# facebookresearch/AVID-CMA

Measured on AMD Instinct MI355X. Metric: clips/sec (video+audio fwd+bwd+NCE+Adam), higher is better.
Workload: dtype f32 (bf16x3 MFMA)

## Files before the change

### avid-cma_amd/avid_hip/lib.py

```python
from __future__ import annotations

import ctypes as C
import os
import subprocess


import torch

_HERE = os.path.dirname(os.path.abspath(__file__))
_PKG = os.path.dirname(_HERE)
LIB_PATH = os.environ.get("AVID_HIP_LIB") or os.path.join(_HERE, "libavid_hip.so")

AVID_OK = 0


class BnBwdFuse(C.Structure):
    _fields_ = [("x", C.c_void_p), ("scale", C.c_void_p), ("shift", C.c_void_p), ("mean", C.c_void_p),
                ("invstd", C.c_void_p), ("relu", C.c_int32), ("partials", C.c_void_p)]


class InAffine(C.Structure):
    _fields_ = [("scale", C.c_void_p), ("shift", C.c_void_p), ("relu", C.c_int32)]


# ... 52 lines not shown
_lib = _load()

_vp, _i, _i64, _u64, _f, _sz = C.c_void_p, C.c_int, C.c_int64, C.c_uint64, C.c_float, C.c_size_t
_dp = C.POINTER(ConvDesc)

SIGNATURES = {
    "avid_last_error": (C.c_char_p, []),
    "avid_version": (_i, []),
    "avid_device_info": (_i, [_i, C.POINTER(_i), C.POINTER(_i), C.c_char_p, _i]),
    "avid_timing_enable": (_i, [_i]),
    "avid_timing_report": (_i, [C.c_char_p, _sz]),
    "avid_conv_fwd_workspace_bytes": (_sz, [_dp]),
    "avid_conv_fwd_stats_rows": (_i, [_dp]),
    "avid_conv_fwd": (_i, [_dp, _vp, _vp, _vp, _vp, _vp, _i, _vp, _vp, _vp, _sz, _vp]),
    "avid_conv_takes_in_affine": (_i, [_dp]),
    "avid_conv_fwd_in": (_i, [_dp, _vp, _vp, _vp, _vp, _vp, _vp, _i, _vp, _vp, _vp, _sz, _vp]),
    "avid_debug_in_affine_launches": (C.c_longlong, [_i]),
    "avid_conv_dgrad_workspace_bytes": (_sz, [_dp]),
    "avid_conv_dgrad_bn_rows": (_i, [_dp]),
    "avid_conv_dgrad": (_i, [_dp, _vp, _vp, _vp, _vp, _vp, _vp, _vp, _vp, _vp, _sz, _vp]),
    "avid_weight_transpose_batched": (_i, [_i, _vp, _i64, _vp]),
    "avid_weight_transform": (_i, [_vp, _vp]),
    "avid_conv_wgrad_workspace_bytes": (_sz, [_dp]),
    "avid_conv_wgrad": (_i, [_dp, _vp, _vp, _vp, _vp, _sz, _vp]),
    "avid_conv_wgrad_in": (_i, [_dp, _vp, _vp, _vp, _vp, _vp, _sz, _vp]),
    "avid_conv_wgrad_groupable": (_i, [_dp]),
    "avid_conv_wgrad_group_workspace_bytes": (_sz, [_i, C.POINTER(WgradItem)]),
    "avid_conv_wgrad_group": (_i, [_i, C.POINTER(WgradItem), _vp, _sz, _vp]),
    "avid_conv_kernel_name": (_i, [_dp, _i, C.c_char_p, _i]),
    "avid_conv_uses_wino": (_i, [_dp, _i]),
    "avid_conv_uses_split": (_i, [_dp, _i]),
    "avid_conv_split_bytes": (_sz, [_dp]),
    "avid_debug_presplit_launches": (C.c_longlong, []),
    "avid_wino_configure": (_i, [_i, _i64, _i]),
    "avid_wino2_configure": (_i, [_i]),
    "avid_wino2_pre_configure": (_i, [_i]),
    "avid_wgrad_pre_configure": (_i, [_i]),
    "avid_stem_fwd_pre_configure": (_i, [_i]),
    "avid_tconv_configure": (_i, [_i]),
    "avid_set_cu_budget": (_i, [_i]),
    "avid_cu_budget": (_i, []),
    "avid_bn_workspace_bytes": (_sz, [_i64, _i]),
    "avid_bn_fwd_train": (_i, [_i64, _i, _vp, _vp, _vp, _vp, _vp, _f, _f, _i, _vp, _vp, _vp, _vp, _vp, _vp, _vp, _i, _vp, _sz, _vp]),
    "avid_bn_fwd_eval": (_i, [_i64, _i, _vp, _vp, _vp, _vp, _vp, _f, _i, _vp, _vp, _vp]),
    "avid_bn_bwd": (_i, [_i64, _i, _vp, _vp, _vp, _vp, _vp, _vp, _vp, _i, _vp, _vp, _vp, _vp, _i, _i, _vp, _sz, _vp]),
    "avid_bn_relu_maxpool_fwd": (_i, [_i, _i, _i, _i, _i, _vp, _vp, _vp, _vp, _vp, _f, _f, _vp, _vp, _vp, _vp, _vp, _vp, _vp,
                                      _vp, _i, _vp, _sz, _vp]),
    "avid_bn_relu_maxpool_bwd": (_i, [_i, _i, _i, _i, _i, _vp, _vp, _vp, _vp, _vp, _vp, _vp, _vp, _vp, _vp, _vp, _vp, _sz,
                                      _vp]),
    "avid_clip_normalize": (_i, [_i, _i, _i, _i, _vp, C.POINTER(_f), C.POINTER(_f), _vp, _vp]),
    "avid_logspec_basis_floats": (_sz, [_i]),
    "avid_logspec_basis": (_i, [_i, _vp, _vp]),
    "avid_logspec_workspace_bytes": (_sz, [_i, _i, _i]),
    "avid_logspec": (_i, [_i, _i, _vp, _i, _i, _i, _vp, _vp, _vp, _f, _vp, _vp, _sz, _vp]),
    "avid_maxpool_hw3s2_fwd": (_i, [_i, _i, _i, _i, _i, _vp, _vp, _vp, _vp]),
    "avid_maxpool_hw3s2_bwd": (_i, [_i, _i, _i, _i, _i, _vp, _vp, _vp, _vp]),
    "avid_global_maxpool_fwd": (_i, [_i, _i, _i, _vp, _vp, _vp, _vp]),
    "avid_global_maxpool_bwd": (_i, [_i, _i, _i, _vp, _vp, _vp, _vp]),
    "avid_relu_bwd": (_i, [_i64, _vp, _vp, _vp, _vp]),
    "avid_colsum": (_i, [_i64, _i, _vp, _vp, _vp]),
    "avid_l2norm_fwd": (_i, [_i, _i, _vp, _vp, _vp, _vp]),
    "avid_l2norm_bwd": (_i, [_i, _i, _vp, _vp, _vp, _vp, _vp]),
    "avid_alias_draw": (_i, [_i64, _i64, _vp, _vp, _i, _u64, _u64, _vp, _vp, _i64, _vp, _vp]),
    "avid_counter_add": (_i, [_vp, _u64, _vp]),
    "avid_bank_scores_fwd": (_i, [_i, _i, _i, _i64, _vp, _vp, _vp, _f, _vp, _vp, _vp, _vp]),
    "avid_bank_scores_bwd": (_i, [_i, _i, _i, _i64, _vp, _vp, _vp, _vp, _f, _i, _vp, _vp]),
# ... 86 lines not shown
```

### avid-cma_amd/csrc/conv.hip

```cpp
#include <math.h>
#include <stdlib.h>

#include <atomic>
#include <type_traits>

#include "common.h"

namespace avid {

typedef unsigned int uintx4 __attribute__((ext_vector_type(4)));

struct ConvArgs {
  const float* __restrict__ src;
  const float* __restrict__ wk;
  int w_row, w_nrec;
  const float* __restrict__ addend;
  const float* __restrict__ bias;
  float* __restrict__ dst;
  float* __restrict__ part;
  int B, Ts, Hs, Ws, Cs;
  int Td, Hd, Wd, Cd;
  int kt, kh, kw;
  int st, sh, sw;
  int pt, ph, pw;
// ... 279 lines not shown

constexpr int EPI_ANY = 15;
#ifdef AVID_PK_TRACE
__device__ long long g_pk_trace[1024 * 64];
extern "C" int avid_debug_pk_trace(long long* host) {
  return (int)hipMemcpyFromSymbol(host, HIP_SYMBOL(g_pk_trace), sizeof(long long) * 1024 * 64);
}
#define PK_STAMP(idx) do { if (threadIdx.x == 0 && (idx) < 32) { g_pk_trace[blockIdx.x * 64 + (idx)] = wall_clock64(); g_pk_trace[blockIdx.x * 64 + 32 + (idx)] = clock64(); } } while (0)
#else
#define PK_STAMP(idx) do {} while (0)
#endif
#ifdef AVID_PK_FP32
constexpr bool PK_SPLIT = false;
#else
constexpr bool PK_SPLIT = true;
#endif
typedef __bf16 pk_bf16x8 __attribute__((ext_vector_type(8)));
typedef unsigned pk_uintx4 __attribute__((ext_vector_type(4)));
template <bool DOT = true>
__device__ __forceinline__ void pk_split8(const floatx4& v0, const floatx4& v1, pk_bf16x8& fh, pk_bf16x8& fm, pk_bf16x8& fl) {
  const float v[8] = {v0[0], v0[1], v0[2], v0[3], v1[0], v1[1], v1[2], v1[3]};
  unsigned h[4], m[4], l[4];
#pragma unroll
  for (int i = 0; i < 4; ++i) {
    if (DOT) split2_bf16_dot(v[2 * i], v[2 * i + 1], h[i], m[i], l[i]);
    else split2_bf16(v[2 * i], v[2 * i + 1], h[i], m[i], l[i]);
  }
  fh = __builtin_bit_cast(pk_bf16x8, pk_uintx4{h[0], h[1], h[2], h[3]});
  fm = __builtin_bit_cast(pk_bf16x8, pk_uintx4{m[0], m[1], m[2], m[3]});
  fl = __builtin_bit_cast(pk_bf16x8, pk_uintx4{l[0], l[1], l[2], l[3]});
}

constexpr int PK_BCH = 2 * 2 * 3 * 1024;
template <int WM, int WN, int TM, int TN, int MODE, bool STRIDED = false, int EPI = EPI_ANY, bool BS = false>
__global__ __launch_bounds__(WM * WN * 64, 2) void igemm_pk_kernel(const ConvArgs p) {
  static_assert(!STRIDED || MODE == 1, "parity classes are a dgrad construct");
  constexpr int NT = WM * WN * 64;
  constexpr int BM = WM * TM * 32, BN = WN * TN * 32;
  constexpr int RPP = NT / 8;
  constexpr int PA = BM / RPP, PB = BN / RPP;
  static_assert(BM % RPP == 0 && BN % RPP == 0, "tile rows must be a multiple of the staging pass");
  static_assert(!BS || (NT == 256 && (BN == 64 || BN == 128) && PK_SPLIT), "pre-split weights: the 4-wave tiles of the split-bf16 build");
  constexpr int BCH = (BN / 64) * PK_BCH;
  constexpr int PB3 = BCH / (NT * 16);
  constexpr bool ASWZ = BS && BN == 128;
  constexpr int ALD = ASWZ ? BK : LDK;
  constexpr int STAGE = BS ? BM * ALD + BCH / 4 : (BM + BN) * LDK;
  extern __shared__ __attribute__((aligned(16))) float smem[];
  typedef const ConvArgs __attribute__((address_space(4)))* KArgs;
  const KArgs kp = (KArgs)__builtin_amdgcn_kernarg_segment_ptr();
  const int tid = threadIdx.x, lane = tid & 63, wave = tid >> 6;
  const int wm = wave / WN, wn = wave % WN;
  const int lrow = tid >> 3, lcol = (tid & 7) * 4;
  const int h = lane >> 5, l31 = lane & 31;
  PK_STAMP(0);

  const int ntn = p.Cd / BN;
  const int G = gridDim.x;
  int slot_;
  if (p.pk_paired) {
    const int per = G >> 4;
    const int xcd = blockIdx.x & 7, pos = blockIdx.x >> 3;
    const int second = pos >= per ? 1 : 0;
    slot_ = second * (G >> 1) + xcd * per + (pos - second * per);
  } else {
    slot_ = (int)xcd_remap(blockIdx.x, G);
  }
  const int slot = __builtin_amdgcn_readfirstlane(slot_);
  const int ntaps = p.kt * p.kh * p.kw;
  const int cpt = p.Cs / BK;
  const int nk = ntaps * cpt;
  const int cs4 = p.Cs * 4;
  const int pix_per_b = p.Ts * p.Hs * p.Ws;
  const int pix_d = p.Td * p.Hd * p.Wd;
  const __amdgpu_buffer_rsrc_t rsB = __builtin_amdgcn_make_buffer_rsrc(
      BS ? const_cast<void*>(p.wsp) : (void*)p.wk, 0, BS ? p.wsp_nrec : p.w_nrec, 0x00020000);

  const int n_full = slot < p.pk_full ? (p.pk_full - slot + G - 1) / G : 0;
  int tslot = slot - p.pk_rot;
  tslot += tslot < 0 ? G : 0;
  const int nseg = n_full + (tslot < p.pk_tail_units ? 1 : 0);
  float cs[TN][2], cq[TN][2];
#pragma unroll
  for (int jj = 0; jj < TN; ++jj) cs[jj][0] = cs[jj][1] = cq[jj][0] = cq[jj][1] = 0.f;
  auto write_stats = [&]() {
    if (!p.stats) return;
    float* red = smem;
// ... 38 lines not shown
      const int local = u - kp->cls_ubegin[c];
      const int lt = local / fc;
      const int piece = local - lt * fc;
      tile = kp->cls_begin[c] + lt;
      const int nkc = kp->cls_nd[c][0] * kp->cls_nd[c][1] * kp->cls_nd[c][2] * cpt;
      const int kps = (nkc + fc - 1) / fc;
      k0 = piece * kps < nkc ? piece * kps : nkc;
      k1 = k0 + kps < nkc ? k0 + kps : nkc;
      split = fc > 1 ? piece : -1;
    } else if (j < n_full) {
      tile = slot + j * G; k0 = 0; k1 = nk; split = -1;
    } else {
      int piece;
      if (p.pk_ws) {
        const int r = tslot / p.pk_ws, mt = tslot - r * p.pk_ws;
        const int nt = r / p.pk_f;
        piece = r - nt * p.pk_f;
        tile = p.pk_full + mt * ntn + nt;
      } else {
        tile = p.pk_full + tslot / p.pk_f;
        piece = tslot % p.pk_f;
      }
      split = p.pk_f > 1 ? piece : -1;
      k0 = piece * p.pk_kps;
      k1 = k0 + p.pk_kps < nk ? k0 + p.pk_kps : nk;
    }
  };

  int ld_seg = 0, ld_ks = 0, ld_kend = 0;
  int ld_dt = 0, ld_dh = 0, ld_dw = 0, ld_c0 = 0, ld_tap = 0;
  int ld_nh = p.kh, ld_nw = p.kw, ld_cls = 0;
  int ld_plo = 0, ld_phi = 0, ld_nrec = 0;
  int ld_soff_a = 0, ld_soff_b = 0;
  unsigned a_base[PA], a_mask[PA], a_cur[PA];
  unsigned b_off[PB];
  floatx4 va[PA], vb[PB];
  pk_uintx4 vb3[PB3];
  int ld_bnt = 0;

  auto range_mask = [](int lo, int hi, int k) -> unsigned {
    lo = lo < 0 ? 0 : lo;
    hi = hi > k - 1 ? k - 1 : hi;
    return hi >= lo ? (2u << hi) - (1u << lo) : 0u;
  };
  auto retap = [&]() {
    const int pixoff = ((ld_dt * p.Hs + ld_dh) * p.Ws + ld_dw) * cs4;
    const unsigned tap_off = (unsigned)(MODE == 0 ? pixoff : -pixoff);
    const unsigned sh_t = ld_dt, sh_h = 8 + ld_dh, sh_w = 16 + ld_dw;
#pragma unroll
    for (int i = 0; i < PA; ++i) {
      const unsigned okb = (a_mask[i] >> sh_t) & (a_mask[i] >> sh_h) & (a_mask[i] >> sh_w) & 1u;
      a_cur[i] = okb ? a_base[i] + tap_off : OOB;
    }
  };
  auto setup_tile = [&](int tile) {
    int c = 0, cT = p.Td, cH = p.Hd, cW = p.Wd, cM = p.M, cpix = pix_d, lt = tile;
    unsigned mgW = p.mgW, mgH = p.mgH, mgT = p.mgT;
    int shW = p.shW, shH = p.shH, shT = p.shT;
    int offt = p.pt, offh = p.ph, offw = p.pw, ndt = p.kt, ndh = p.kh, ndw = p.kw;
    if (STRIDED) {
      c = ld_cls;
      lt = tile - kp->cls_begin[c];
      cT = kp->cls_n[c][0]; cH = kp->cls_n[c][1]; cW = kp->cls_n[c][2];
      cpix = cT * cH * cW;
      cM = p.B * cpix;
      mgT = kp->cls_mg[c][0]; mgH = kp->cls_mg[c][1]; mgW = kp->cls_mg[c][2];
      shT = kp->cls_shf[c][0]; shH = kp->cls_shf[c][1]; shW = kp->cls_shf[c][2];
      offt = (kp->cls_p0[c][0] + p.pt - kp->cls_d0[c][0]) / p.st;
      offh = (kp->cls_p0[c][1] + p.ph - kp->cls_d0[c][1]) / p.sh;
      offw = (kp->cls_p0[c][2] + p.pw - kp->cls_d0[c][2]) / p.sw;
      ndt = kp->cls_nd[c][0]; ndh = kp->cls_nd[c][1]; ndw = kp->cls_nd[c][2];
    }
    const int mt = lt / ntn, nt = lt - mt * ntn;
    const int m0 = mt * BM, n0 = nt * BN;
    int b_lo = m0 / cpix;
    if (b_lo >= p.B) b_lo = p.B - 1;
    b_lo = __builtin_amdgcn_readfirstlane(b_lo);
    {
      const long long base = (long long)b_lo * pix_per_b * p.Cs;
      long long a_bytes = ((long long)p.B * pix_per_b * p.Cs - base) * 4;
      if (a_bytes > 0x7fffffffll) a_bytes = 0x7fffffffll;
      const unsigned long long ptr = reinterpret_cast<unsigned long long>(p.src + base);
      ld_plo = __builtin_amdgcn_readfirstlane((int)(unsigned)ptr);
      ld_phi = __builtin_amdgcn_readfirstlane((int)(unsigned)(ptr >> 32));
      ld_nrec = __builtin_amdgcn_readfirstlane((int)a_bytes);
    }
    static_assert(PA <= 8, "one decoded row per lane of an 8-lane staging group");
    unsigned dec_base, dec_mask;
    {
      const int i = (tid & 7) % PA;
      const unsigned m = m0 + lrow + RPP * i;
      const bool ok = m < (unsigned)cM;
      const unsigned mm = ok ? m : 0u;
      const unsigned q1 = magic_div(mm, mgW, shW);
      const int wd = mm - q1 * cW;
      const unsigned q2 = magic_div(q1, mgH, shH);
      const int hd = q1 - q2 * cH;
      const int b = magic_div(q2, mgT, shT);
      const int td = q2 - b * cT;
      int t0, h0, w0;
      unsigned mt_, mh, mw;
      if (MODE == 0) {
        t0 = td * p.st - p.pt; h0 = hd * p.sh - p.ph; w0 = wd * p.sw - p.pw;
        mt_ = range_mask(-t0, p.Ts - 1 - t0, p.kt);
        mh = range_mask(-h0, p.Hs - 1 - h0, p.kh);
        mw = range_mask(-w0, p.Ws - 1 - w0, p.kw);
      } else {
        t0 = td + offt; h0 = hd + offh; w0 = wd + offw;
        mt_ = range_mask(t0 - p.Ts + 1, t0, ndt);
        mh = range_mask(h0 - p.Hs + 1, h0, ndh);
        mw = range_mask(w0 - p.Ws + 1, w0, ndw);
      }
      dec_mask = ok ? (mt_ | (mh << 8) | (mw << 16)) : 0u;
      dec_base = (unsigned)((((b - b_lo) * p.Ts + t0) * p.Hs + h0) * p.Ws + w0) * cs4;
    }
#pragma unroll
    for (int i = 0; i < PA; ++i) {
      const int src = (lane & ~7) | i;
      a_mask[i] = (unsigned)__shfl((int)dec_mask, src, 64);
      a_base[i] = (unsigned)__shfl((int)dec_base, src, 64) + lcol * 4;
    }
#pragma unroll
    for (int i = 0; i < PB; ++i) b_off[i] = (unsigned)((n0 + lrow + RPP * i) * p.w_row + lcol) * 4;
    if (BS) ld_bnt = __builtin_amdgcn_readfirstlane(nt * BCH);
  };
  auto issue_loads = [&]() {
    const unsigned long long ptr = ((unsigned long long)(unsigned)__builtin_amdgcn_readfirstlane(ld_phi) << 32) |
                                   (unsigned)__builtin_amdgcn_readfirstlane(ld_plo);
    const __amdgpu_buffer_rsrc_t rsA = __builtin_amdgcn_make_buffer_rsrc(
        reinterpret_cast<void*>(ptr), 0, __builtin_amdgcn_readfirstlane(ld_nrec), 0x00020000);
    const int soff_a = __builtin_amdgcn_readfirstlane(ld_soff_a);
    const int soff_b = __builtin_amdgcn_readfirstlane(ld_soff_b);
#pragma unroll
    for (int i = 0; i < PA; ++i)
      va[i] = __builtin_bit_cast(floatx4, __builtin_amdgcn_raw_buffer_load_b128(rsA, a_cur[i], soff_a, 0));
    if (BS) {
      const int soff_b3 = __builtin_amdgcn_readfirstlane(ld_soff_b + ld_bnt);
#pragma unroll
      for (int i = 0; i < PB3; ++i)
        vb3[i] = __builtin_bit_cast(pk_uintx4, __builtin_amdgcn_raw_buffer_load_b128(rsB, (tid + NT * i) * 16, soff_b3, 0));
      return;
    }
#pragma unroll
    for (int i = 0; i < PB; ++i)
      vb[i] = __builtin_bit_cast(floatx4, __builtin_amdgcn_raw_buffer_load_b128(rsB, b_off[i], soff_b, 0));
  };
  const auto sgpr = [](int v) { return __builtin_amdgcn_readfirstlane(v); };
  auto set_tap = [&]() {
    if (STRIDED) {
      const int c = ld_cls;
      ld_tap = sgpr(((kp->cls_d0[c][0] + ld_dt * p.st) * p.kh + kp->cls_d0[c][1] + ld_dh * p.sh) * p.kw + kp->cls_d0[c][2] +
                    ld_dw * p.sw);
    } else {
      ld_tap = sgpr((ld_dt * p.kh + ld_dh) * p.kw + ld_dw);
    }
    ld_soff_a = sgpr(ld_c0 * 4);
    ld_soff_b = BS ? sgpr((ld_tap * cpt + ld_c0 / BK) * p.wsp_kstep) : sgpr((ld_tap * p.Cs + ld_c0) * 4);
  };
  auto setup_seg = [&](int j) {
    int tile, k0, k1, split;
    seg_info(j, tile, k0, k1, split);
    if (STRIDED) {
      while (k1 == k0 && j + 1 < nseg) seg_info(++j, tile, k0, k1, split);
      ld_seg = sgpr(k1 == k0 ? nseg : j);
      if (k1 == k0) return;
      ld_cls = sgpr(cls_of(tile));
      ld_nh = sgpr(kp->cls_nd[ld_cls][1]);
// ... 21 lines not shown
        moved = ld_seg < nseg;
      }
    } else if (ld_c0 != p.Cs) {
      ld_soff_a = sgpr(ld_soff_a + BK * 4);
      ld_soff_b = sgpr(ld_soff_b + (BS ? p.wsp_kstep : BK * 4));
    } else {
      ld_c0 = 0;
      int dw = ld_dw + 1, dh = ld_dh, dt = ld_dt;
      if (dw == ld_nw) { dw = 0; ++dh; }
      if (dh == ld_nh) { dh = 0; ++dt; }
      ld_dw = sgpr(dw);
      ld_dh = sgpr(dh);
      ld_dt = sgpr(dt);
      set_tap();
      moved = true;
    }
    if (moved) retap();
  };
  auto store_stage = [&](float* st) {
#pragma unroll
    for (int i = 0; i < PA; ++i)
      *reinterpret_cast<floatx4*>(&st[(lrow + RPP * i) * ALD + (ASWZ ? (((tid & 7) ^ ((lrow >> 1) & 7)) << 2) : lcol)]) = va[i];
    if (BS) {
#pragma unroll
      for (int i = 0; i < PB3; ++i)
        *reinterpret_cast<pk_uintx4*>(reinterpret_cast<char*>(st + BM * ALD) + (tid + NT * i) * 16) = vb3[i];
      return;
    }
#pragma unroll
    for (int i = 0; i < PB; ++i) *reinterpret_cast<floatx4*>(&st[(BM + lrow + RPP * i) * LDK + lcol]) = vb[i];
  };

  setup_seg(0);
  if (!STRIDED || ld_seg < nseg) {
    retap();
    issue_loads();
    advance();
    store_stage(smem);
    if (ld_seg < nseg) {
      issue_loads();
      advance();
    }
  }
  __syncthreads();
  PK_STAMP(1);

  const int a_frag = (wm * TM * 32 + l31) * LDK + h * 4;
  const int b_frag = (BM + wn * TN * 32 + l31) * LDK + h * 4;
  int left = n_full * nk;
  if (STRIDED) {
    left = 0;
    for (int j = 0; j < nseg; ++j) {
      int tile, k0, k1, split;
      seg_info(j, tile, k0, k1, split);
      left += k1 - k0;
    }
  } else if (nseg > n_full) {
    int tile, k0, k1, split;
    seg_info(n_full, tile, k0, k1, split);
    left += k1 - k0;
  }
  int u = 0;
  floatx16 acc[TM][TN];

  auto ktile = [&](auto ST, auto LD) {
    const float* cur = smem + u * STAGE;
    float* nxt = smem + (u ^ 1) * STAGE;
    const float* Ab = cur + a_frag;
    const float* Bb = cur + b_frag;
    if (BS) {
      const float* As = ASWZ ? cur + (wm * TM * 32 + l31) * ALD : Ab - h * 4 + h * 8;
      const int akey = (l31 >> 1) & 7;
      const char* Bc = reinterpret_cast<const char*>(cur + BM * ALD) + lane * 16;
      floatx4 ar[2][TM][2];
      pk_bf16x8 bq[2][TN][3];
      auto fetch = [&](int st, int slot) {
        const int o0 = ASWZ ? (((st * 4 + h * 2) ^ akey) << 2) : st * 16;
        const int o1 = ASWZ ? (((st * 4 + h * 2 + 1) ^ akey) << 2) : st * 16 + 4;
#pragma unroll
        for (int i = 0; i < TM; ++i) {
          ar[slot][i][0] = *reinterpret_cast<const floatx4*>(As + i * 32 * ALD + o0);
          ar[slot][i][1] = *reinterpret_cast<const floatx4*>(As + i * 32 * ALD + o1);
        }
#pragma unroll
        for (int j = 0; j < TN; ++j) {
          const char* Bj = Bc + (((wn * TN + j) * 2 + st) * 3) * 1024;
          bq[slot][j][0] = *reinterpret_cast<const pk_bf16x8*>(Bj);
          bq[slot][j][1] = *reinterpret_cast<const pk_bf16x8*>(Bj + 1024);
          bq[slot][j][2] = *reinterpret_cast<const pk_bf16x8*>(Bj + 2048);
        }
      };
#ifdef AVID_PK_PREFETCH
      constexpr bool PF = TM * TN <= 2 && !STRIDED;
#else
      constexpr bool PF = false;
#endif
// ... 88 lines not shown
      if (decltype(ST)::value && g == 0) {
#pragma unroll
        for (int q = 0; q < PA + PB; ++q) {
          __builtin_amdgcn_sched_group_barrier(0x008, 1, 0);
          __builtin_amdgcn_sched_group_barrier(0x200, 1, 0);
        }
      }
      if (decltype(LD)::value && g == 1) {
#pragma unroll
        for (int q = 0; q < PA + PB; ++q) {
          __builtin_amdgcn_sched_group_barrier(0x008, 1, 0);
          __builtin_amdgcn_sched_group_barrier(0x020, 1, 0);
        }
      }
      __builtin_amdgcn_sched_barrier(0);
    }
  };

  const int row_bytes = p.Cd * 4;
  for (int j = 0; j < nseg; ++j) {
    int tile, k0, k1, split;
    seg_info(j, tile, k0, k1, split);
    const int nkj = k1 - k0;
#pragma unroll
    for (int i = 0; i < TM; ++i)
#pragma unroll
      for (int jj = 0; jj < TN; ++jj)
#pragma unroll
        for (int r = 0; r < 16; ++r) acc[i][jj][r] = 0.f;

    int nst = left - 2 < nkj ? left - 2 : nkj;
    if (nst < 0) nst = 0;
    PK_STAMP(2 + 3 * j);
    for (int ks = 0; ks < nst; ++ks, u ^= 1) {
      ktile(std::true_type{}, std::true_type{});
      advance();
      __syncthreads();
    }
    left -= nst;
    if (nst < nkj) {
      if (left == 2) {
        ktile(std::true_type{}, std::false_type{});
        __syncthreads();
        u ^= 1;
        --left;
        ++nst;
      }
      if (nst < nkj) {
        ktile(std::false_type{}, std::false_type{});
        __syncthreads();
        u ^= 1;
        --left;
      }
    }

    PK_STAMP(3 + 3 * j);
    if (STRIDED) {
      int* drow = reinterpret_cast<int*>(smem + 2 * STAGE);
      int* arow = drow + BM;
      const bool sparse_add = p.add_s[0] * p.add_s[1] * p.add_s[2] > 1;
      const int c = cls_of(tile);
      const int lt = tile - kp->cls_begin[c];
      const int mt = lt / ntn, nt = lt - mt * ntn;
      const int n0 = nt * BN;
      const int cT = kp->cls_n[c][0], cH = kp->cls_n[c][1], cW = kp->cls_n[c][2];
      __syncthreads();
      if (tid < BM) {
        const unsigned m = mt * BM + tid;
        const bool ok = m < (unsigned)(p.B * cT * cH * cW);
        const unsigned mm = ok ? m : 0u;
        const unsigned q1 = magic_div(mm, kp->cls_mg[c][2], kp->cls_shf[c][2]);
        const int wd = mm - q1 * cW;
        const unsigned q2 = magic_div(q1, kp->cls_mg[c][1], kp->cls_shf[c][1]);
        const int hd = q1 - q2 * cH;
        const int b = magic_div(q2, kp->cls_mg[c][0], kp->cls_shf[c][0]);
        const int td = q2 - b * cT;
        const int dst = ((b * p.Td + kp->cls_p0[c][0] + td * p.st) * p.Hd + kp->cls_p0[c][1] + hd * p.sh) * p.Wd +
                        kp->cls_p0[c][2] + wd * p.sw;
        drow[tid] = ok ? dst * row_bytes : (int)OOB;
        if (sparse_add) {
          const int t = kp->cls_p0[c][0] + td * p.st, hh = kp->cls_p0[c][1] + hd * p.sh, w = kp->cls_p0[c][2] + wd * p.sw;
          const bool on = ok && (t & (p.add_s[0] - 1)) == 0 && (hh & (p.add_s[1] - 1)) == 0 && (w & (p.add_s[2] - 1)) == 0;
          const int ar = ((b * p.add_n[0] + (t >> (p.add_s[0] - 1))) * p.add_n[1] + (hh >> (p.add_s[1] - 1))) * p.add_n[2] +
                         (w >> (p.add_s[2] - 1));
          arow[tid] = on ? ar * row_bytes : (int)OOB;
        } else {
          arow[tid] = ok ? dst * row_bytes : (int)OOB;
        }
      }
      __syncthreads();
      const bool direct = split < 0;
// ... 105 lines not shown
      }
    };
    constexpr std::true_type Y{};
    constexpr std::false_type N{};
    constexpr std::integral_constant<int, 0> ADD{};
    constexpr std::integral_constant<int, 0> B0{};
    constexpr std::integral_constant<int, 1> B1{};
    constexpr std::integral_constant<int, 2> BQ{};
    if (!direct) emit(N, N, N, ADD, N, B0);
    else if (EPI == 0) emit(Y, N, N, ADD, N, B0);
    else if (EPI == 1) emit(Y, Y, N, ADD, N, B0);
    else if (MODE == 0 && EPI == 2) emit(Y, N, N, ADD, N, B1);
    else if (MODE == 0 && EPI == 3) emit(Y, N, Y, ADD, N, B1);
    else if (MODE == 0 && EPI == 4) emit(Y, Y, N, std::integral_constant<int, 1>{}, N, B0);
    else if (MODE == 0 && EPI == 5) emit(Y, Y, N, std::integral_constant<int, 2>{}, N, B0);
    else if (MODE == 1 && EPI == 8) emit(Y, N, N, ADD, Y, B0);
    else if (MODE == 1 && EPI == 9) emit(Y, Y, N, ADD, Y, B0);
    else if (MODE == 1 && p.bnb_x) {
      if (p.addend) emit(Y, Y, N, ADD, Y, BQ); else emit(Y, N, N, ADD, Y, BQ);
    } else if (p.addend) {
      if (MODE == 0 && p.epi_op == 1) emit(Y, Y, N, std::integral_constant<int, 1>{}, N, BQ);
      else if (MODE == 0 && p.epi_op == 2) emit(Y, Y, N, std::integral_constant<int, 2>{}, N, BQ);
      else if (p.relu) emit(Y, Y, Y, ADD, N, BQ);
      else emit(Y, Y, N, ADD, N, BQ);
    } else {
      if (p.relu) emit(Y, N, Y, ADD, N, BQ); else emit(Y, N, N, ADD, N, BQ);
    }
    PK_STAMP(4 + 3 * j);
  }
  write_stats();
  PK_STAMP(31);
}

constexpr int WG_LD_C = 64 + 4;
constexpr int TC_P = 32;
constexpr int TC_T = 8;
constexpr int TC_ROWS = TC_P * TC_T;
constexpr int TC_B_BYTES = 6 * PK_BCH;
constexpr int TC_STAGE = TC_ROWS * LDK;
constexpr size_t TC_LDS = TC_B_BYTES + (2 * TC_STAGE + TC_P * LDK + 128) * sizeof(float);

template <int MODE, int EPI, bool AFF = false>
__global__ __launch_bounds__(512) __attribute__((amdgpu_waves_per_eu(2, 2))) void tconv64_kernel(const ConvArgs p) {
  static_assert(!AFF || MODE == 0, "the input affine map belongs to the forward");
  extern __shared__ __attribute__((aligned(16))) float smem[];
  char* Bs = reinterpret_cast<char*>(smem);
  float* As = smem + TC_B_BYTES / 4;
  const int tid = threadIdx.x, lane = tid & 63;
  const int wave = __builtin_amdgcn_readfirstlane(tid >> 6);
  const int h = lane >> 5, l31 = lane & 31;
  const int lcol = (tid & 7) * 4;
  const int G = gridDim.x;
  const int slot = __builtin_amdgcn_readfirstlane((int)xcd_remap(blockIdx.x, G));
  PK_STAMP(0);
  const int HW = p.Hs * p.Ws;
  const int NP = p.B * HW;
  const int ntiles = (NP + TC_P - 1) / TC_P;
  const int nmine = slot < ntiles ? (ntiles - slot + G - 1) / G : 0;
  const int nitems = 2 * nmine;
  const int frame_bytes = HW * 256;

  float cs[2][2], cq[2][2];
#pragma unroll
  for (int j = 0; j < 2; ++j) cs[j][0] = cs[j][1] = cq[j][0] = cq[j][1] = 0.f;
  auto write_stats = [&]() {
    if (!p.stats) return;
// ... 1769 lines not shown
}
constexpr int S2_WIDE_DEFAULT = 0;
static int bs_wide_mode() {
  static int v = -1;
  if (v < 0) {
    const char* e = getenv("AVID_BS_WIDE");
    v = e ? atoi(e) : 2;
    if (v < 0 || v > 2) v = 2;
  }
  return v;
}
static bool bs_rows() {
  static int v = -1;
  if (v < 0) {
    const char* e = getenv("AVID_BS_ROWS");
    v = e ? (atoi(e) != 0 ? 1 : 0) : 1;
  }
  return v != 0;
}
static bool s2_wide() {
  static std::atomic<int> v{-1};
  int m = v.load(std::memory_order_relaxed);
  if (m < 0) {
    const char* e = getenv("AVID_S2_WIDE");
    m = e ? (atoi(e) != 0 ? 1 : 0) : S2_WIDE_DEFAULT;
    v.store(m, std::memory_order_relaxed);
  }
  return m != 0;
}
static bool bs_wide(const PkPlan& pk) { return pk.tile == 0 && (bs_wide_mode() == 2 || (bs_wide_mode() == 1 && pk.full == 0)); }

static std::atomic<long long> g_presplit_launches{0};

template <int WM, int WN, int TM, int TN, int MODE, bool STRIDED, int EPI>
static void launch_pk_e(const ConvArgs& a, int grid, size_t lds, hipStream_t s) {
  if constexpr (pk_takes_split<WM, WN, TM, TN, EPI>() && !(STRIDED && WN == 2)) {
    if (a.wsp) {
      ++g_presplit_launches;
      constexpr int BM = WM * TM * 32, BN = WN * TN * 32;
      const size_t lds3 = sizeof(float) * 2 * (BM * (BN == 128 ? BK : LDK) + (BN / 64) * PK_BCH / 4) + (STRIDED ? sizeof(int) * 2 * BM : 0);
      launch_pk_eb<WM, WN, TM, TN, MODE, STRIDED, EPI, true>(a, grid, lds3, s);
      return;
    }
  }
  launch_pk_eb<WM, WN, TM, TN, MODE, STRIDED, EPI, false>(a, grid, lds, s);
}

template <int WM, int WN, int TM, int TN, int MODE, bool STRIDED = false>
static int launch_pk(const ConvArgs& a, int grid, hipStream_t s) {
  constexpr int BM = WM * TM * 32, BN = WN * TN * 32;
  const size_t lds = sizeof(float) * 2 * (BM + BN) * LDK + (STRIDED ? sizeof(int) * 2 * BM : 0);
  static char name[64] = "";
  if (!name[0]) snprintf(name, sizeof(name), "igemm_pk_kernel<%d,%d,%d,%d,%d>%s", WM, WN, TM, TN, MODE, STRIDED ? "s2" : "");
  const double K = (double)a.kt * a.kh * a.kw * a.Cs;
  const double srcpix = (double)a.B * a.Ts * a.Hs * a.Ws;
  const double flops = MODE == 1 ? 2.0 * srcpix * a.Cd * K : 2.0 * a.M * a.Cd * K;
  ScopedTimer t(s, name, flops,
                4.0 * (srcpix * a.Cs + (double)a.Cd * K + (double)a.M * a.Cd * (1 + (a.addend ? 1 : 0) + (a.bnb_x ? 1 : 0))));
  constexpr bool MAIN = (WM * WN == 4) || (WM == 2 && WN == 1);
  const int epi = MAIN ? epi_code<MODE>(a) : EPI_ANY;
  switch (epi) {
    case 0: launch_pk_e<WM, WN, TM, TN, MODE, STRIDED, MAIN ? 0 : EPI_ANY>(a, grid, lds, s); break;
    case 1: launch_pk_e<WM, WN, TM, TN, MODE, STRIDED, MAIN ? 1 : EPI_ANY>(a, grid, lds, s); break;
    case 2: launch_pk_e<WM, WN, TM, TN, MODE, STRIDED, (MAIN && MODE == 0 && !STRIDED) ? 2 : EPI_ANY>(a, grid, lds, s); break;
    case 3: launch_pk_e<WM, WN, TM, TN, MODE, STRIDED, (MAIN && MODE == 0 && !STRIDED) ? 3 : EPI_ANY>(a, grid, lds, s); break;
    case 4: launch_pk_e<WM, WN, TM, TN, MODE, STRIDED, (MAIN && MODE == 0 && !STRIDED) ? 4 : EPI_ANY>(a, grid, lds, s); break;
    case 5: launch_pk_e<WM, WN, TM, TN, MODE, STRIDED, (MAIN && MODE == 0 && !STRIDED) ? 5 : EPI_ANY>(a, grid, lds, s); break;
    case 8: launch_pk_e<WM, WN, TM, TN, MODE, STRIDED, (MAIN && MODE == 1) ? 8 : EPI_ANY>(a, grid, lds, s); break;
    case 9: launch_pk_e<WM, WN, TM, TN, MODE, STRIDED, (MAIN && MODE == 1) ? 9 : EPI_ANY>(a, grid, lds, s); break;
    default: launch_pk_e<WM, WN, TM, TN, MODE, STRIDED, EPI_ANY>(a, grid, lds, s); break;
  }
  return check_launch("igemm_pk");
// ... 457 lines not shown
  a.bnb_relu = 0;
  a.mgW = a.mgH = a.mgT = 0; a.shW = a.shH = a.shT = 0;
  a.add_s[0] = a.add_s[1] = a.add_s[2] = 1;
  a.add_n[0] = a.add_n[1] = a.add_n[2] = 0;
  a.wsp = nullptr;
  a.wsp_nrec = a.wsp_kstep = 0;
  a.stats_rows = 0;
  return dispatch_igemm<0>(a, nullptr, 0, s);
}

}

using namespace avid;

static bool conv_takes_split(const avid_conv_desc* d, int which) {
#ifdef AVID_NO_PRESPLIT
  return false;
#endif
  if (!PK_SPLIT || d->x_channel_first) return false;
  if (which == 0) {
    if (d->Cin % 32 || d->Cout % 64 || wino_supported(d, 0)) return false;
    const long long M = (long long)d->B * d->To * d->Ho * d->Wo;
    const PkPlan pk = plan_pk(M, d->Cout, trim_taps(d).d.kt * d->kh * d->kw * (d->Cin / BK), 0);
    return pk.tile == 1 || bs_wide(pk);
  }
  if (d->Cin % 64 || d->Cout % 32 || d->st > 2 || d->sh > 2 || d->sw > 2 || wino_supported(d, 1)) return false;
  const long long M = (long long)d->B * d->Ti * d->Hi * d->Wi;
  if (d->st > 1 || d->sh > 1 || d->sw > 1) return M * d->Cin * 4 < (1ll << 31) && (d->Cin % 128 != 0 || !s2_wide());
  const PkPlan pk = plan_pk(M, d->Cin, trim_taps(d).d.kt * d->kh * d->kw * (d->Cout / BK), 1);
  return pk.tile == 1 || bs_wide(pk);
}

extern "C" long long avid_debug_presplit_launches(void) { return g_presplit_launches.load(std::memory_order_relaxed); }

extern "C" int avid_tconv_configure(int mode) {
  g_tconv_mode.store((mode >= 0 && mode <= 2) ? mode : -1, std::memory_order_relaxed);
  return tconv_mode();
}

extern "C" int avid_conv_uses_split(const avid_conv_desc* d, int which) {
  if (!d || validate(d) || which < 0 || which > 1) return 0;
  return conv_takes_split(d, which) ? 1 : 0;
}

extern "C" size_t avid_conv_split_bytes(const avid_conv_desc* d) {
  if (!d || validate(d)) return 0;
  return (size_t)6 * d->Cout * d->kt * d->kh * d->kw * d->Cin;
}

static void set_split_operand(ConvArgs& a, const void* planes, int N, int C, int ntaps_full, int khw, int dt0) {
  const int kstep = (N / 64) * PK_BCH;
  const long long off = (long long)dt0 * khw * (C / BK) * kstep, total = (long long)ntaps_full * (C / BK) * kstep;
  a.wsp = static_cast<const char*>(planes) + off;
  a.wsp_nrec = (int)(total - off);
  a.wsp_kstep = kstep;
}

extern "C" size_t avid_conv_fwd_workspace_bytes(const avid_conv_desc* d) {
  if (!d || validate(d)) return 0;
  const bool vec = (d->Cin % 32 == 0) && !d->x_channel_first;
  if (!vec) return stem_fwd_supported(d) ? stem_fwd_ws_bytes(d) : 0;
  const long long M = (long long)d->B * d->To * d->Ho * d->Wo;
  const Trim tr = trim_taps(d);
  const int nk = tr.d.kt * d->kh * d->kw * (d->Cin / BK);
  size_t need = sizeof(float) * igemm_ws_floats(M, d->Cout, nk, 0);
  if (wino_supported(d, 0) && wino_ws_bytes(d, 0) > need) need = wino_ws_bytes(d, 0);
// ... 727 lines not shown
```

### include/avid_hip.h

```cpp
#ifndef AVID_HIP_H
#define AVID_HIP_H

#include <stddef.h>
#include <stdint.h>

#ifdef __cplusplus
extern "C" {
#endif

#define AVID_OK 0
#define AVID_E_BADARG (-1)
#define AVID_E_SHAPE (-2)
#define AVID_E_HIP (-3)
#define AVID_E_UNSUPPORTED (-4)

typedef void* avid_stream_t;

const char* avid_last_error(void);
int avid_version(void);
int avid_device_info(int device, int* cu_count, int* lds_bytes, char* arch, int arch_len);

int avid_timing_enable(int on);
int avid_timing_report(char* buf, size_t len);

// ... 22 lines not shown
                     const float* addend, const float* bias, int relu, float* y, float* bn_partials, void* ws, size_t ws_bytes,
                     avid_stream_t stream);
long long avid_debug_in_affine_launches(int fused);

size_t avid_conv_dgrad_workspace_bytes(const avid_conv_desc* d);
typedef struct {
  const float* x;
  const float* scale;
  const float* shift;
  const float* mean;
  const float* invstd;
  int32_t relu;
  float* partials;
} avid_bn_bwd_fuse;
int avid_conv_dgrad_bn_rows(const avid_conv_desc* d);
int avid_conv_dgrad(const avid_conv_desc* d, const float* dy, const float* w, const float* wt, const float* u,
                    const float* addend, const int32_t* addend_stride, float* dx, const avid_bn_bwd_fuse* bn,
                    void* ws, size_t ws_bytes, avid_stream_t stream);

typedef struct avid_wt_desc {
  const float* w;
  float* wt;
  int32_t Cout, ntaps, Cin;
  int32_t mode;
} avid_wt_desc;
int avid_weight_transpose_batched(int n, const avid_wt_desc* descs_dev, int64_t max_elems, avid_stream_t stream);
int avid_weight_transform(const avid_wt_desc* desc, avid_stream_t stream);

int avid_conv_kernel_name(const avid_conv_desc* d, int which, char* buf, int len);
int avid_conv_uses_wino(const avid_conv_desc* d, int which);
int avid_conv_uses_split(const avid_conv_desc* d, int which);
size_t avid_conv_split_bytes(const avid_conv_desc* d);
long long avid_debug_presplit_launches(void);

int avid_wino_configure(int enabled, int64_t min_pixels, int max_channels);
int avid_wino2_configure(int min_rounds_x10);
int avid_wino2_pre_configure(int on);
int avid_wgrad_pre_configure(int on);
int avid_stem_fwd_pre_configure(int on);

int avid_tconv_configure(int mode);

int avid_set_cu_budget(int cus);
int avid_cu_budget(void);

size_t avid_conv_wgrad_workspace_bytes(const avid_conv_desc* d);
int avid_conv_wgrad(const avid_conv_desc* d, const float* x, const float* dy, float* dw, void* ws,
                    size_t ws_bytes, avid_stream_t stream);
int avid_conv_wgrad_in(const avid_conv_desc* d, const float* x, const avid_in_affine* in, const float* dy, float* dw, void* ws,
                       size_t ws_bytes, avid_stream_t stream);

typedef struct avid_wgrad_item {
  avid_conv_desc d;
  const float* x;
  const float* dy;
  float* dw;
} avid_wgrad_item;
int avid_conv_wgrad_groupable(const avid_conv_desc* d);
size_t avid_conv_wgrad_group_workspace_bytes(int n, const avid_wgrad_item* items);
int avid_conv_wgrad_group(int n, const avid_wgrad_item* items, void* ws, size_t ws_bytes, avid_stream_t stream);

size_t avid_bn_workspace_bytes(int64_t M, int C);
int avid_bn_fwd_train(int64_t M, int C, const float* x, const float* gamma, const float* beta,
                      float* running_mean, float* running_var, float momentum, float eps, int relu,
                      float* y, float* save_mean, float* save_invstd, float* save_scale,
                      float* save_shift, int64_t* num_batches_tracked, const float* partials, int nparts,
// ... 160 lines not shown
```

Measured before the change: 6979.

## Stage implicit-GEMM operands via LDS-DMA buffer loads into a two-slot ring

Adds a DMA variant of the pre-split bf16x3 implicit-GEMM conv kernel that uses buffer_load ... lds to write activation and pre-split weight tiles straight into a double-buffered LDS ring. This skips the register round-trip and the explicit store_stage. Activation rows are written with an XOR swizzle so the fragment reads avoid bank conflicts. The path is on by default for the 4x1 wave tiles (TN 2 or 4) and can be turned off with AVID_PK_DMA. In exchange it relies on inline asm that manipulates m0 and on vmcnt waits, and each k-tile now needs a full barrier.

```diff
diff --git a/avid-cma_amd/avid_hip/lib.py b/avid-cma_amd/avid_hip/lib.py
--- a/avid-cma_amd/avid_hip/lib.py
+++ b/avid-cma_amd/avid_hip/lib.py
@@ -108,6 +108,7 @@
     "avid_conv_uses_split": (_i, [_dp, _i]),
     "avid_conv_split_bytes": (_sz, [_dp]),
     "avid_debug_presplit_launches": (C.c_longlong, []),
+    "avid_debug_pk_dma_launches": (C.c_longlong, []),
     "avid_wino_configure": (_i, [_i, _i64, _i]),
     "avid_wino2_configure": (_i, [_i]),
     "avid_wino2_pre_configure": (_i, [_i]),
diff --git a/avid-cma_amd/csrc/conv.hip b/avid-cma_amd/csrc/conv.hip
--- a/avid-cma_amd/csrc/conv.hip
+++ b/avid-cma_amd/csrc/conv.hip
@@ -335,14 +335,32 @@
 }
 
 constexpr int PK_BCH = 2 * 2 * 3 * 1024;
-template <int WM, int WN, int TM, int TN, int MODE, bool STRIDED = false, int EPI = EPI_ANY, bool BS = false>
-__global__ __launch_bounds__(WM * WN * 64, 2) void igemm_pk_kernel(const ConvArgs p) {
+constexpr int PK_RING = 2;
+template <int BN>
+constexpr int pk_slot() { return 128 * BK + (BN / 64) * PK_BCH / 4; }
+typedef int pk_intx4 __attribute__((ext_vector_type(4)));
+__device__ __forceinline__ void pk_dma16(pk_intx4 rs, unsigned voff, int soff, int lds) {
+  unsigned keep;
+  asm volatile("s_mov_b32 %0, m0\n\ts_mov_b32 m0, %4\n\ts_nop 0\n\tbuffer_load_dwordx4 %1, %2, %3 offen lds\n\ts_mov_b32 m0, %0"
+               : "=&s"(keep) : "v"(voff), "s"(rs), "s"(soff), "s"(lds) : "memory");
+}
+__device__ __forceinline__ unsigned pk_lds_addr(const void* q) { return (unsigned)(size_t)q; }
+template <int N>
+__device__ __forceinline__ void pk_ring_wait() {
+  asm volatile("s_waitcnt vmcnt(%0)\n\ts_waitcnt lgkmcnt(0)\n\ts_barrier" ::"i"(N) : "memory");
+}
+template <int WM, int WN, int TM, int TN, int MODE, bool STRIDED, int EPI, bool BS, bool DMA>
+__device__ __forceinline__ void igemm_pk_body(const ConvArgs& p) {
   static_assert(!STRIDED || MODE == 1, "parity classes are a dgrad construct");
+  static_assert(!DMA || (BS && WM == 4 && WN == 1 && TM == 1 && (TN == 2 || TN == 4)), "the LDS-DMA ring: the four-wave pre-split tiles");
   constexpr int NT = WM * WN * 64;
   constexpr int BM = WM * TM * 32, BN = WN * TN * 32;
   constexpr int RPP = NT / 8;
   constexpr int PA = BM / RPP, PB = BN / RPP;
   static_assert(BM % RPP == 0 && BN % RPP == 0, "tile rows must be a multiple of the staging pass");
+  constexpr int PAL = PA;
+  constexpr int AGS = 8;
+  constexpr int ARS = RPP;
   static_assert(!BS || (NT == 256 && (BN == 64 || BN == 128) && PK_SPLIT), "pre-split weights: the 4-wave tiles of the split-bf16 build");
   constexpr int BCH = (BN / 64) * PK_BCH;
   constexpr int PB3 = BCH / (NT * 16);
@@ -356,6 +374,8 @@
   const int wm = wave / WN, wn = wave % WN;
   const int lrow = tid >> 3, lcol = (tid & 7) * 4;
   const int h = lane >> 5, l31 = lane & 31;
+  const int arow0 = lrow;
+  const int acol_b = DMA ? (((tid & 7) ^ ((lrow >> 1) & 7)) << 4) : lcol * 4;
   PK_STAMP(0);
 
   const int ntn = p.Cd / BN;
@@ -460,7 +480,7 @@
   int ld_nh = p.kh, ld_nw = p.kw, ld_cls = 0;
   int ld_plo = 0, ld_phi = 0, ld_nrec = 0;
   int ld_soff_a = 0, ld_soff_b = 0;
-  unsigned a_base[PA], a_mask[PA], a_cur[PA];
+  unsigned a_base[PAL], a_mask[PAL], a_cur[PAL];
   unsigned b_off[PB];
   floatx4 va[PA], vb[PB];
   pk_uintx4 vb3[PB3];
@@ -476,7 +496,7 @@
     const unsigned tap_off = (unsigned)(MODE == 0 ? pixoff : -pixoff);
     const unsigned sh_t = ld_dt, sh_h = 8 + ld_dh, sh_w = 16 + ld_dw;
 #pragma unroll
-    for (int i = 0; i < PA; ++i) {
+    for (int i = 0; i < PAL; ++i) {
       const unsigned okb = (a_mask[i] >> sh_t) & (a_mask[i] >> sh_h) & (a_mask[i] >> sh_w) & 1u;
       a_cur[i] = okb ? a_base[i] + tap_off : OOB;
     }
@@ -513,11 +533,11 @@
       ld_phi = __builtin_amdgcn_readfirstlane((int)(unsigned)(ptr >> 32));
       ld_nrec = __builtin_amdgcn_readfirstlane((int)a_bytes);
     }
-    static_assert(PA <= 8, "one decoded row per lane of an 8-lane staging group");
+    static_assert(PAL <= AGS, "one decoded row per lane of a staging group");
     unsigned dec_base, dec_mask;
     {
-      const int i = (tid & 7) % PA;
-      const unsigned m = m0 + lrow + RPP * i;
+      const int i = (tid & (AGS - 1)) % PAL;
+      const unsigned m = m0 + arow0 + ARS * i;
       const bool ok = m < (unsigned)cM;
       const unsigned mm = ok ? m : 0u;
       const unsigned q1 = magic_div(mm, mgW, shW);
@@ -543,10 +563,10 @@
       dec_base = (unsigned)((((b - b_lo) * p.Ts + t0) * p.Hs + h0) * p.Ws + w0) * cs4;
     }
 #pragma unroll
-    for (int i = 0; i < PA; ++i) {
-      const int src = (lane & ~7) | i;
+    for (int i = 0; i < PAL; ++i) {
+      const int src = (lane & ~(AGS - 1)) | i;
       a_mask[i] = (unsigned)__shfl((int)dec_mask, src, 64);
-      a_base[i] = (unsigned)__shfl((int)dec_base, src, 64) + lcol * 4;
+      a_base[i] = (unsigned)__shfl((int)dec_base, src, 64) + acol_b;
     }
 #pragma unroll
     for (int i = 0; i < PB; ++i) b_off[i] = (unsigned)((n0 + lrow + RPP * i) * p.w_row + lcol) * 4;
@@ -560,7 +580,7 @@
     const int soff_a = __builtin_amdgcn_readfirstlane(ld_soff_a);
     const int soff_b = __builtin_amdgcn_readfirstlane(ld_soff_b);
 #pragma unroll
-    for (int i = 0; i < PA; ++i)
+    for (int i = 0; i < PAL; ++i)
       va[i] = __builtin_bit_cast(floatx4, __builtin_amdgcn_raw_buffer_load_b128(rsA, a_cur[i], soff_a, 0));
     if (BS) {
       const int soff_b3 = __builtin_amdgcn_readfirstlane(ld_soff_b + ld_bnt);
@@ -648,17 +668,21 @@
   };
 
   setup_seg(0);
-  if (!STRIDED || ld_seg < nseg) {
-    retap();
-    issue_loads();
-    advance();
-    store_stage(smem);
-    if (ld_seg < nseg) {
+  if constexpr (!DMA) {
+    if (!STRIDED || ld_seg < nseg) {
+      retap();
       issue_loads();
       advance();
-    }
-  }
-  __syncthreads();
+      store_stage(smem);
+      if (ld_seg < nseg) {
+        issue_loads();
+        advance();
+      }
+    }
+    __syncthreads();
+  } else if (!STRIDED || ld_seg < nseg) {
+    retap();
+  }
   PK_STAMP(1);
 
   const int a_frag = (wm * TM * 32 + l31) * LDK + h * 4;
@@ -678,6 +702,79 @@
   }
   int u = 0;
   floatx16 acc[TM][TN];
+
+  constexpr int SLOT = pk_slot<BN>();
+  const int left0 = left;
+  int q_issued = 0;
+  int l_slot = 0, r_slot = 0;
+  const int wv = sgpr(wave);
+  auto dma_issue = [&]() {
+    if constexpr (DMA) {
+      const pk_intx4 rsA = {sgpr(ld_plo), sgpr(ld_phi), sgpr(ld_nrec), 0x00020000};
+      const unsigned long long wp = reinterpret_cast<unsigned long long>(p.wsp);
+      const pk_intx4 rsW = {sgpr((int)(unsigned)wp), sgpr((int)(unsigned)(wp >> 32)), sgpr(p.wsp_nrec), 0x00020000};
+      const int base = sgpr((int)pk_lds_addr(smem + l_slot * SLOT));
+      const int soff_a = sgpr(ld_soff_a);
+#pragma unroll
+      for (int i = 0; i < PA; ++i) pk_dma16(rsA, a_cur[i], soff_a, sgpr(base + (wv * 8 + RPP * i) * BK * 4));
+      const int soff_w = sgpr(ld_soff_b + ld_bnt);
+      static_assert(BCH == PB3 * 4 * 1024 && NT == 256, "PB3 weight kilobytes per wave");
+#pragma unroll
+      for (int m = 0; m < PB3; ++m) pk_dma16(rsW, lane * 16, sgpr(soff_w + (wv + 4 * m) * 1024), sgpr(base + (BM * BK + (wv + 4 * m) * 256) * 4));
+      l_slot ^= 1;
+      ++q_issued;
+      advance();
+    }
+  };
+  auto ring_wait = [&](bool after_epi) {
+    if constexpr (DMA) {
+      constexpr int E = 16 * TM * TN < 63 ? 16 * TM * TN : 63;
+      if (after_epi) pk_ring_wait<E>();
+      else pk_ring_wait<0>();
+    }
+  };
+  auto ktile_dma = [&]() {
+    const float* As = smem + r_slot * SLOT + (wm * TM * 32 + l31) * BK;
+    const int akey = (l31 >> 1) & 7;
+    const char* Bc = reinterpret_cast<const char*>(smem + r_slot * SLOT + BM * BK) + lane * 16;
+#pragma unroll
+    for (int st = 0; st < BK / 16; ++st) {
+      floatx4 ar[TM][2];
+      pk_bf16x8 bq[TN][3];
+#pragma unroll
+      for (int i = 0; i < TM; ++i) {
+        ar[i][0] = *reinterpret_cast<const floatx4*>(As + i * 32 * BK + (((st * 4 + h * 2) ^ akey) << 2));
+        ar[i][1] = *reinterpret_cast<const floatx4*>(As + i * 32 * BK + (((st * 4 + h * 2 + 1) ^ akey) << 2));
+      }
+#pragma unroll
+      for (int j = 0; j < TN; ++j) {
+        const char* Bj = Bc + (((wn * TN + j) * 2 + st) * 3) * 1024;
+        bq[j][0] = *reinterpret_cast<const pk_bf16x8*>(Bj);
+        bq[j][1] = *reinterpret_cast<const pk_bf16x8*>(Bj + 1024);
+        bq[j][2] = *reinterpret_cast<const pk_bf16x8*>(Bj + 2048);
+      }
+      pk_bf16x8 ah[TM], am[TM], al[TM];
+#pragma unroll
+      for (int i = 0; i < TM; ++i) pk_split8(ar[i][0], ar[i][1], ah[i], am[i], al[i]);
+#pragma unroll
+      for (int j = 0; j < TN; ++j) {
+        const pk_bf16x8 bh = bq[j][0], bm = bq[j][1], bl = bq[j][2];
+#pragma unroll
+        for (int i = 0; i < TM; ++i) {
+          acc[i][j] = __builtin_amdgcn_mfma_f32_32x32x16_bf16(ah[i], bl, acc[i][j], 0, 0, 0);
+          acc[i][j] = __builtin_amdgcn_mfma_f32_32x32x16_bf16(al[i], bh, acc[i][j], 0, 0, 0);
+          acc[i][j] = __builtin_amdgcn_mfma_f32_32x32x16_bf16(am[i], bm, acc[i][j], 0, 0, 0);
+          acc[i][j] = __builtin_amdgcn_mfma_f32_32x32x16_bf16(ah[i], bm, acc[i][j], 0, 0, 0);
+          acc[i][j] = __builtin_amdgcn_mfma_f32_32x32x16_bf16(am[i], bh, acc[i][j], 0, 0, 0);
+          acc[i][j] = __builtin_amdgcn_mfma_f32_32x32x16_bf16(ah[i], bh, acc[i][j], 0, 0, 0);
+        }
+      }
+    }
+    r_slot ^= 1;
+  };
+  if constexpr (DMA) {
+    if (left > 0) dma_issue();
+  }
 
   auto ktile = [&](auto ST, auto LD) {
     const float* cur = smem + u * STAGE;
@@ -832,31 +929,39 @@
     int nst = left - 2 < nkj ? left - 2 : nkj;
     if (nst < 0) nst = 0;
     PK_STAMP(2 + 3 * j);
-    for (int ks = 0; ks < nst; ++ks, u ^= 1) {
-      ktile(std::true_type{}, std::true_type{});
-      advance();
-      __syncthreads();
-    }
-    left -= nst;
-    if (nst < nkj) {
-      if (left == 2) {
-        ktile(std::true_type{}, std::false_type{});
+    if constexpr (DMA) {
+      for (int kt = 0; kt < nkj; ++kt) {
+        ring_wait(j > 0 && kt == 0);
+        if (q_issued < left0) dma_issue();
+        ktile_dma();
+      }
+    } else {
+      for (int ks = 0; ks < nst; ++ks, u ^= 1) {
+        ktile(std::true_type{}, std::true_type{});
+        advance();
         __syncthreads();
-        u ^= 1;
-        --left;
-        ++nst;
-      }
+      }
+      left -= nst;
       if (nst < nkj) {
-        ktile(std::false_type{}, std::false_type{});
-        __syncthreads();
-        u ^= 1;
-        --left;
+        if (left == 2) {
+          ktile(std::true_type{}, std::false_type{});
+          __syncthreads();
+          u ^= 1;
+          --left;
+          ++nst;
+        }
+        if (nst < nkj) {
+          ktile(std::false_type{}, std::false_type{});
+          __syncthreads();
+          u ^= 1;
+          --left;
+        }
       }
     }
 
     PK_STAMP(3 + 3 * j);
     if (STRIDED) {
-      int* drow = reinterpret_cast<int*>(smem + 2 * STAGE);
+      int* drow = reinterpret_cast<int*>(smem + (DMA ? PK_RING * pk_slot<BN>() : 2 * STAGE));
       int* arow = drow + BM;
       const bool sparse_add = p.add_s[0] * p.add_s[1] * p.add_s[2] > 1;
       const int c = cls_of(tile);
@@ -1028,6 +1133,15 @@
   PK_STAMP(31);
 }
 
+template <int WM, int WN, int TM, int TN, int MODE, bool STRIDED = false, int EPI = EPI_ANY, bool BS = false>
+__global__ __launch_bounds__(WM * WN * 64, 2) void igemm_pk_kernel(const ConvArgs p) {
+  igemm_pk_body<WM, WN, TM, TN, MODE, STRIDED, EPI, BS, false>(p);
+}
+template <int WM, int WN, int TM, int TN, int MODE, bool STRIDED, int EPI>
+__global__ __launch_bounds__(WM * WN * 64, 2) void igemm_pk_dma_kernel(const ConvArgs p) {
+  igemm_pk_body<WM, WN, TM, TN, MODE, STRIDED, EPI, true, true>(p);
+}
+
 constexpr int WG_LD_C = 64 + 4;
 constexpr int TC_P = 32;
 constexpr int TC_T = 8;
@@ -2863,12 +2977,38 @@
 
 static std::atomic<long long> g_presplit_launches{0};
 
+static bool pk_dma() {
+  static std::atomic<int> v{-1};
+  int m = v.load(std::memory_order_relaxed);
+  if (m < 0) {
+    const char* e = getenv("AVID_PK_DMA");
+    m = e ? (atoi(e) != 0 ? 1 : 0) : 1;
+    v.store(m, std::memory_order_relaxed);
+  }
+  return m != 0;
+}
+static std::atomic<long long> g_pk_dma_launches{0};
+
 template <int WM, int WN, int TM, int TN, int MODE, bool STRIDED, int EPI>
 static void launch_pk_e(const ConvArgs& a, int grid, size_t lds, hipStream_t s) {
   if constexpr (pk_takes_split<WM, WN, TM, TN, EPI>() && !(STRIDED && WN == 2)) {
     if (a.wsp) {
       ++g_presplit_launches;
       constexpr int BM = WM * TM * 32, BN = WN * TN * 32;
+      if constexpr (WM == 4 && WN == 1 && TM == 1 && (TN == 2 || TN == 4)) {
+        if (pk_dma()) {
+          ++g_pk_dma_launches;
+          static bool attr_set = false;
+          auto kern = igemm_pk_dma_kernel<WM, WN, TM, TN, MODE, STRIDED, EPI>;
+          const size_t ldsd = sizeof(float) * PK_RING * pk_slot<BN>() + (STRIDED ? sizeof(int) * 2 * BM : 0);
+          if (!attr_set) {
+            (void)hipFuncSetAttribute(reinterpret_cast<const void*>(kern), hipFuncAttributeMaxDynamicSharedMemorySize, (int)ldsd);
+            attr_set = true;
+          }
+          hipLaunchKernelGGL(kern, dim3(grid), dim3(WM * WN * 64), ldsd, s, a);
+          return;
+        }
+      }
       const size_t lds3 = sizeof(float) * 2 * (BM * (BN == 128 ? BK : LDK) + (BN / 64) * PK_BCH / 4) + (STRIDED ? sizeof(int) * 2 * BM : 0);
       launch_pk_eb<WM, WN, TM, TN, MODE, STRIDED, EPI, true>(a, grid, lds3, s);
       return;
@@ -3392,6 +3532,7 @@
 }
 
 extern "C" long long avid_debug_presplit_launches(void) { return g_presplit_launches.load(std::memory_order_relaxed); }
+extern "C" long long avid_debug_pk_dma_launches(void) { return g_pk_dma_launches.load(std::memory_order_relaxed); }
 
 extern "C" int avid_tconv_configure(int mode) {
   g_tconv_mode.store((mode >= 0 && mode <= 2) ? mode : -1, std::memory_order_relaxed);
diff --git a/include/avid_hip.h b/include/avid_hip.h
--- a/include/avid_hip.h
+++ b/include/avid_hip.h
@@ -78,6 +78,7 @@
 int avid_conv_uses_split(const avid_conv_desc* d, int which);
 size_t avid_conv_split_bytes(const avid_conv_desc* d);
 long long avid_debug_presplit_launches(void);
+long long avid_debug_pk_dma_launches(void);
 
 int avid_wino_configure(int enabled, int64_t min_pixels, int max_channels);
 int avid_wino2_configure(int min_rounds_x10);
```

Result: no change. 6995 (median of 6 runs) (+0.2%).
